# mom-ocean/MOM6

Measured on AMD Instinct MI355X. Metric: simulated-days/wall-sec, higher is better.
Workload: dtype f64

## Files before the change

### mom6_amd/abi.py

```python
import ctypes as C
import os

_HERE = os.path.dirname(os.path.abspath(__file__))
LIB_PATH = os.path.join(_HERE, "lib", "libmom6x.so")

c_double_p = C.POINTER(C.c_double)


class Dims(C.Structure):
    _fields_ = [
        ("ni", C.c_int), ("nj", C.c_int), ("nk", C.c_int), ("halo", C.c_int),
        ("ioff", C.c_int), ("joff", C.c_int), ("pitch", C.c_int), ("slab", C.c_int),
        ("i_glob0", C.c_int), ("j_glob0", C.c_int), ("ni_glob", C.c_int), ("nj_glob", C.c_int),
        ("reentrant_x", C.c_int), ("reentrant_y", C.c_int),
    ]

    @property
    def nrows(self):
        return self.nj + 2 * self.halo + 1

    def shape2(self):
        return (self.nrows, self.pitch)

    def shape3(self, nk=None):
# ... 387 lines not shown
    g_prime = np.empty(nk)
    g_prime[0] = g_Earth
    g_prime[1:] = (g_Earth / Rho0) * (Rlay[1:] - Rlay[:-1])
    return np.ascontiguousarray(Rlay), np.ascontiguousarray(g_prime)


class RK2Params(C.Structure):
    _fields_ = [("be", C.c_double), ("begw", C.c_double), ("split_bottom_stress", C.c_int),
                ("BT_use_layer_fluxes", C.c_int), ("store_CAu", C.c_int), ("visc_rem_dt_bug", C.c_int), ("remap_aux", C.c_int),
                ("no_BT_cont", C.c_int)]


def rk2_params_default():
    p = RK2Params()
    p.be, p.begw = 0.6, 0.0
    p.split_bottom_stress = 0
    p.BT_use_layer_fluxes = p.store_CAu = p.visc_rem_dt_bug = 1
    p.remap_aux = 0
    p.no_BT_cont = 0
    return p


VERTVISC_COEF_HOOK = C.CFUNCTYPE(C.c_int, C.c_void_p, C.c_int, C.c_void_p, C.c_void_p, C.c_void_p, C.c_double)
HOR_VISC_HOOK = C.CFUNCTYPE(C.c_int, C.c_void_p, C.c_void_p, C.c_void_p, C.c_void_p, C.c_void_p, C.c_void_p,
                            C.c_void_p, C.c_void_p)


class RK2Hooks(C.Structure):
    _fields_ = [("user", C.c_void_p), ("vertvisc_coef", VERTVISC_COEF_HOOK), ("horizontal_viscosity", HOR_VISC_HOOK)]


RK2_FIELDS = ["CAu", "CAv", "CAu_pred", "CAv_pred", "PFu", "PFv", "diffu", "diffv", "visc_rem_u", "visc_rem_v",
              "u_accel_bt", "v_accel_bt", "u_av", "v_av", "h_av", "pbce", "eta", "eta_PF", "uhbt", "vhbt",
              "taux_bot", "tauy_bot", "BT_h_u", "BT_h_v"]
RK2_HAVE_ETA, RK2_HAVE_DIFFU, RK2_HAVE_U2, RK2_HAVE_CAU, RK2_HAVE_UH, RK2_HAVE_H2 = 1, 2, 4, 8, 16, 32
RK2_FIELDS_2D = {"eta", "eta_PF", "uhbt", "vhbt", "taux_bot", "tauy_bot"}


METRICS = [
    "mask2dT", "mask2dCu", "mask2dCv", "mask2dBu",
    "dxT", "dyT", "IdxT", "IdyT",
    "dxCu", "dyCu", "IdxCu", "IdyCu",
    "dxCv", "dyCv", "IdxCv", "IdyCv",
    "dxBu", "dyBu", "IdxBu", "IdyBu",
    "areaT", "IareaT", "areaBu", "IareaBu",
    "areaCu", "areaCv", "IareaCu", "IareaCv",
    "dy_Cu", "dx_Cv", "bathyT", "CoriolisBu", "Coriolis2Bu",
]
G = {n: i for i, n in enumerate(METRICS)}
G_COUNT = len(METRICS)

MOM6X_OK = 0

_lib = None


ABI_VERSION = 6


def load_library(path=None):
    global _lib
    if _lib is not None and path is None:
        return _lib
    p = path or LIB_PATH
    if not os.path.exists(p):
        raise RuntimeError(
            f"mom6_amd: HIP extension {p} is missing; run `python -c 'import __graft_entry__ as g; g.build()'`. "
            "There is no CPU fallback for the product path.")
    lib = C.CDLL(p, mode=C.RTLD_GLOBAL)
# ... 24 lines not shown
```

### mom6_amd/csrc/continuity.hip

```cpp
#include "continuity_dev.h"
#include "continuity_lds.h"
#include <cstdlib>

namespace {

bool use_lds_path(int nk) {
  const char *e = getenv("MOM6X_MASSFLUX");
  if (e && !strcmp(e, "legacy")) return false;
  return mass_flux_lds_usable(nk);
}


template <int DIR>
__global__ void __launch_bounds__(256)
k_edge(Dm d, const double *__restrict__ G, const double *__restrict__ h_in, double *__restrict__ h_L,
       double *__restrict__ h_R, double h_min, int scheme , int monotonic,
       int i0, int i1, int j0, int j1) {
  const int i = i0 + blockIdx.x * blockDim.x + threadIdx.x;
  const int j = j0 + blockIdx.y * blockDim.y + threadIdx.y;
  const int k = blockIdx.z;
  if (i > i1 || j > j1) return;
  const int st = DIR ? d.pitch : 1;
  const double *m = gm(G, d, MOM6X_G_mask2dT);
  const size_t c2 = ix2(d, i, j);
// ... 244 lines not shown
  const int j = b0 + blockIdx.y * blockDim.y + threadIdx.y;
  const int k = blockIdx.z;
  if (i > a1 || j > b1) return;
  const int st = DIR ? d.pitch : 1;
  const double *IdT = gm(G, d, DIR ? MOM6X_G_IdyT : MOM6X_G_IdxT);
  const double *Lface = gm(G, d, DIR ? MOM6X_G_dx_Cv : MOM6X_G_dy_Cu), *IareaT = gm(G, d, MOM6X_G_IareaT);
  const size_t f2 = ix2(d, i, j), f = f2 + (size_t)k * d.slab, p = f + st;
  const double uf = u[f];
  double h_avg, h_marg;
  if (uf > 0.0) {
    const double CFL = vol_CFL ? (uf * dt) * (Lface[f2] * IareaT[f2]) : uf * dt * IdT[f2];
    const double curv_3 = (hL[f] + hR[f]) - 2.0 * h[f];
    h_avg = hR[f] + CFL * (0.5 * (hL[f] - hR[f]) + curv_3 * (CFL - 1.5));
    h_marg = hR[f] + CFL * ((hL[f] - hR[f]) + 3.0 * curv_3 * (CFL - 1.0));
  } else if (uf < 0.0) {
    const double CFL = vol_CFL ? (-uf * dt) * (Lface[f2] * IareaT[f2 + st]) : -uf * dt * IdT[f2 + st];
    const double curv_3 = (hL[p] + hR[p]) - 2.0 * h[p];
    h_avg = hL[p] + CFL * (0.5 * (hR[p] - hL[p]) + curv_3 * (CFL - 1.5));
    h_marg = hL[p] + CFL * ((hR[p] - hL[p]) + 3.0 * curv_3 * (CFL - 1.0));
  } else {
    h_avg = 0.5 * (hL[p] + hR[f]);
    h_marg = 0.5 * (hL[p] + hR[f]);
  }
  double hu = marginal ? h_marg : h_avg;
  if (visc_rem) hu = hu * (visc_rem[f] * 1.0);
  else hu = hu * 1.0;
  h_u[f] = hu;
}

template <int DIR>
__global__ void __launch_bounds__(256)
k_convergence(Dm d, const double *__restrict__ G, double *h, const double *__restrict__ uh, double dt,
              const double *hin, double h_min, int i0, int i1, int j0, int j1, int *flag, double *h_av, const double *av_src,
              int av_mode) {
  const int i = I_BASE(i0) + blockIdx.x * blockDim.x + threadIdx.x;
  const int j = j0 + blockIdx.y * blockDim.y + threadIdx.y;
  if (i < i0 || i > i1 || j > j1) return;
  const int st = DIR ? d.pitch : 1;
  const size_t c2 = ix2(d, i, j), slab = (size_t)d.slab;
  const double IareaT = gm(G, d, MOM6X_G_IareaT)[c2];
  const int k0 = blockIdx.z * KCHUNK, k1 = min(k0 + KCHUNK, d.nk);
  const bool own = (i >= 0 && i <= d.ni - 1 && j >= 0 && j <= d.nj - 1);
  bool bad = false;
  for (int k = k0; k < k1; k++) {
    const size_t c = c2 + (size_t)k * slab;
    const double h_old = hin[c];
    const double hn = h_old - dt * IareaT * (uh[c] - uh[c - st]);
    const double hnew = dmax(hn, h_min);
    h[c] = hnew;
    if (av_mode && own) {
      if (av_mode == 1) h_av[c] = 0.5 * (av_src[c] + hnew);
      else if (av_mode == 2) h_av[c] = h_old;
      else h_av[c] = 0.5 * (h_av[c] + hnew);
    }
    bad = bad || (hn != hn);
  }
  if (bad) atomicOr(flag, 1);
}

template <int DIR>
int run_direction(mom6x_ctx *c, const double *u, const double *h_src, double *h, double *uh, double dt,
                  int ish, int ieh, int jsh, int jeh, const double *uhbt, const double *visc_rem,
                  double *u_cor, const mom6x_BT_cont *BT, double *du_cor, const double *hin_conv,
                  double h_min_conv, bool first_pass) {
  const Dm d = c->d;
  const mom6x_continuity_params &P = c->cont;
  const dim3 blk(64, 4, 1);
  int ei0 = ish, ei1 = ieh, ej0 = jsh, ej1 = jeh;
  if (DIR == 0) { ei0 = ish - 1; ei1 = ieh + 1; } else { ej0 = jsh - 1; ej1 = jeh + 1; }
  const int scheme = P.upwind_1st ? 2 : (P.simple_2nd ? 1 : 0);
  const bool special = P.aggress_adjust || P.vol_CFL;
  const bool wave = !special && (P.sum_order == MOM6X_SUM_TREE16 || P.sum_order == MOM6X_SUM_TREE16_FMA);
  const bool lds = !special && (wave || use_lds_path(d.nk));
  if (!lds)
    KLAUNCH(c, "k_edge<DIR>", k_edge<DIR>, grid3(ei1 - ei0 + 1, ej1 - ej0 + 1, d.nk, blk), blk, d, c->G, h_src,
                       c->hL, c->hR, 2.0 * c->GV.Angstrom_H, scheme, P.monotonic, ei0, ei1, ej0, ej1);
  FluxArgs A;
  memset(&A, 0, sizeof(A));
  A.u = u; A.h_in = h_src; A.hL = c->hL; A.hR = c->hR; A.uh = uh; A.uhbt = uhbt; A.visc_rem = visc_rem;
  A.u_cor = u_cor; A.du_cor = du_cor; A.set_BT_cont = (BT != nullptr);
  if (BT) {
    if (DIR == 0) { A.FA_m0 = BT->FA_u_W0; A.FA_mm = BT->FA_u_WW; A.uBT_mm = BT->uBT_WW;
                    A.FA_p0 = BT->FA_u_E0; A.FA_pp = BT->FA_u_EE; A.uBT_pp = BT->uBT_EE; }
    else          { A.FA_m0 = BT->FA_v_S0; A.FA_mm = BT->FA_v_SS; A.uBT_mm = BT->vBT_SS;
                    A.FA_p0 = BT->FA_v_N0; A.FA_pp = BT->FA_v_NN; A.uBT_pp = BT->vBT_NN; }
  }
  A.dt = dt; A.CFL_limit_adjust = P.CFL_limit_adjust; A.tol_eta = P.tol_eta; A.tol_vel = P.tol_vel;
  A.better_iter = P.better_iter; A.use_visc_rem_max = P.use_visc_rem_max;
  A.aggress_adjust = P.aggress_adjust; A.vol_CFL = P.vol_CFL;
// ... 18 lines not shown
      FluxArgs S1 = A, S2 = A;
      S1.a0 = a0; S1.a1 = a1; S1.b0 = b0; S1.b1 = b1;
      S2.a0 = c0; S2.a1 = c1; S2.b0 = e0; S2.b1 = e1;
      return mass_flux_wave_pair(c, DIR, S1, S2, E);
    };
    int rc;
    if (!split) {
      rc = part(A.a0, A.a1, A.b0, A.b1);
    } else if (DIR == 0) {
      const int o0 = A.b0 > 0 ? A.b0 : 0, o1 = A.b1 < d.nj - 1 ? A.b1 : d.nj - 1;
      rc = part(A.a0, A.a1, o0, o1);
      halo_complete(c);
      if (!rc) rc = pair(A.a0, A.a1, A.b0, o0 - 1, A.a0, A.a1, o1 + 1, A.b1);
    } else {
      const int o0 = A.a0 > 0 ? A.a0 : 0, o1 = A.a1 < d.ni - 1 ? A.a1 : d.ni - 1;
      rc = part(o0, o1, A.b0, A.b1);
      halo_complete(c);
      if (!rc) rc = pair(A.a0, o0 - 1, A.b0, A.b1, o1 + 1, A.a1, A.b0, A.b1);
    }
    if (rc) return rc;
  } else {
    KLAUNCH(c, "k_mass_flux<DIR>", k_mass_flux<DIR>, grid3(A.a1 - A.a0 + 1, A.b1 - A.b0 + 1, 1, blk), blk, d, c->G, A);
    if (BT_h) {
      KLAUNCH(c, "k_flux_thickness<DIR>", k_flux_thickness<DIR>, grid3(A.a1 - A.a0 + 1, A.b1 - A.b0 + 1, d.nk, blk), blk,
                         d, c->G, (u_cor ? (const double *)u_cor : u), h_src, c->hL, c->hR, BT_h, dt,
                         P.marginal_faces, visc_rem, A.a0, A.a1, A.b0, A.b1, P.vol_CFL);
    }
  }
  if (first_pass || !c->cont_h_unused)
  {
    int av_mode = 0;
    if (c->cont_av_kind == 1 && !first_pass) av_mode = 1;
    if (c->cont_av_kind == 2) av_mode = first_pass ? 2 : 3;
    KLAUNCH(c, "k_convergence<DIR>", k_convergence<DIR>, grid3(nxa(ieh - ish + 1, ish), jeh - jsh + 1, nchunks(d.nk), blk), blk, d, c->G,
                       h, uh, dt, hin_conv, h_min_conv, ish, ieh, jsh, jeh, c->flag, c->cont_av, c->cont_av_src, av_mode);
  }
  HIPCHK(hipGetLastError());
  return MOM6X_OK;
}

}

extern "C" int mom6x_continuity_init(mom6x_ctx *c, const mom6x_continuity_params *p) {
  REQUIRE(c && p, MOM6X_EINVAL, "mom6x_continuity_init: null argument");
  REQUIRE(p->sum_order == MOM6X_SUM_REFERENCE || p->sum_order == MOM6X_SUM_TREE16 || p->sum_order == MOM6X_SUM_TREE16_FMA, MOM6X_EINVAL,
          "continuity_PPM: sum_order must be MOM6X_SUM_REFERENCE (0), MOM6X_SUM_TREE16 (1) or MOM6X_SUM_TREE16_FMA (2)");
  REQUIRE(p->sum_order == MOM6X_SUM_REFERENCE || mass_flux_wave_usable(c->d.nk), MOM6X_EUNSUPPORTED,
          "continuity_PPM: sum_order = MOM6X_SUM_TREE16(_FMA) carries at most 128 layers; use MOM6X_SUM_REFERENCE");
  c->cont = *p;
  c->cont_init = true;
  return MOM6X_OK;
}

extern "C" int mom6x_continuity_stats(mom6x_ctx *c, int mode, unsigned long long *out3) {
  REQUIRE(c, MOM6X_EINVAL, "mom6x_continuity_stats: null context");
  const int reset = (mode == 1);
  if (mode == 1) c->cont_stats_on = true;
  if (mode == 0) c->cont_stats_on = false;
  HIPCHK(hipSetDevice(c->device));
  if (!c->cont_stats) {
    HIPCHK(hipMalloc(&c->cont_stats, 4 * sizeof(unsigned long long)));
    HIPCHK(hipMemsetAsync(c->cont_stats, 0, 4 * sizeof(unsigned long long), c->stream));
  }
  HIPCHK(hipStreamSynchronize(c->stream));
  if (out3) HIPCHK(hipMemcpy(out3, c->cont_stats, 3 * sizeof(unsigned long long), hipMemcpyDeviceToHost));
  if (reset) HIPCHK(hipMemsetAsync(c->cont_stats, 0, 4 * sizeof(unsigned long long), c->stream));
  return MOM6X_OK;
}
// ... 35 lines not shown
```

### mom6_amd/csrc/dyn_split_RK2.hip

```cpp
#include <algorithm>
#include <cstring>
#include "mom6x_dev.h"

void halo_wrap(mom6x_ctx *c, double *const *fields, const int *staggers, const int *nks, int n);

struct RK2State {
  mom6x_rk2_params P;
  double *CAu, *CAv, *CAu_pred, *CAv_pred, *PFu, *PFv, *diffu, *diffv, *visc_rem_u, *visc_rem_v;
  double *u_accel_bt, *v_accel_bt, *u_av, *v_av, *h_av, *pbce;
  double *eta, *eta_PF, *uhbt, *vhbt, *taux_bot, *tauy_bot;
  mom6x_BT_cont BT;
  bool CAu_pred_stored;
  bool accel_bt_deferred;
  double *up, *vp, *hp, *u_bc_accel, *v_bc_accel, *uh_in, *vh_in, *eta_pred, *eta_h;
};

namespace {

__global__ void __launch_bounds__(256)
k_bc_accel(Dm d, const double *__restrict__ G, const double *__restrict__ CAu, const double *__restrict__ CAv,
           const double *__restrict__ PFu, const double *__restrict__ PFv, const double *__restrict__ diffu,
           const double *__restrict__ diffv, double *__restrict__ u_bc, double *__restrict__ v_bc,
           const double *__restrict__ u, const double *__restrict__ v, double *__restrict__ up, double *__restrict__ vp,
           double dt) {
// ... 160 lines not shown
}

extern "C" int mom6x_initialize_dyn_split_RK2(mom6x_ctx *c, const mom6x_rk2_params *p) {
  REQUIRE(c && p, MOM6X_EINVAL, "mom6x_initialize_dyn_split_RK2: null argument");
  REQUIRE(c->cont_init && c->bt_init && c->cor_init && c->pgf_init, MOM6X_EINVAL,
          "initialize_dyn_split_RK2: continuity, barotropic, CoriolisAdv and PressureForce must be initialised first");
  REQUIRE(!p->remap_aux || p->store_CAu, MOM6X_EINVAL, "REMAP_AUXILIARY_VARS requires that STORE_CORIOLIS_ACCEL = True.");
  REQUIRE(p->BT_use_layer_fluxes && p->store_CAu, MOM6X_EUNSUPPORTED,
          "dyn_split_RK2: only BT_USE_LAYER_FLUXES=True and STORE_CORIOLIS_ACCEL=True are supported");
  HIPCHK(hipSetDevice(c->device));
  if (c->rk2) rk2_state_free(c);
  RK2State *s = new RK2State();
  memset(s, 0, sizeof(*s));
  s->P = *p;
  const size_t n2 = (size_t)c->dims.slab, n3 = n2 * c->dims.nk;
  double **p3[] = { &s->CAu, &s->CAv, &s->CAu_pred, &s->CAv_pred, &s->PFu, &s->PFv, &s->diffu, &s->diffv, &s->visc_rem_u,
                    &s->visc_rem_v, &s->u_accel_bt, &s->v_accel_bt, &s->u_av, &s->v_av, &s->h_av, &s->pbce, &s->up, &s->vp,
                    &s->hp, &s->u_bc_accel, &s->v_bc_accel, &s->uh_in, &s->vh_in, &s->BT.h_u, &s->BT.h_v };
  for (double **q : p3) { HIPCHK(hipMalloc(q, n3 * sizeof(double))); HIPCHK(hipMemsetAsync(*q, 0, n3 * sizeof(double), c->stream)); }
  double **p2[] = { &s->eta, &s->eta_PF, &s->uhbt, &s->vhbt, &s->taux_bot, &s->tauy_bot, &s->eta_pred, &s->eta_h, &s->BT.FA_u_EE,
                    &s->BT.FA_u_E0, &s->BT.FA_u_W0, &s->BT.FA_u_WW, &s->BT.uBT_WW, &s->BT.uBT_EE, &s->BT.FA_v_NN, &s->BT.FA_v_N0,
                    &s->BT.FA_v_S0, &s->BT.FA_v_SS, &s->BT.vBT_SS, &s->BT.vBT_NN };
  for (double **q : p2) { HIPCHK(hipMalloc(q, n2 * sizeof(double))); HIPCHK(hipMemsetAsync(*q, 0, n2 * sizeof(double), c->stream)); }
  s->CAu_pred_stored = false;
  c->rk2 = s;
  return MOM6X_OK;
}

extern "C" double *mom6x_rk2_field(mom6x_ctx *c, int which) {
  if (!c || !c->rk2) return nullptr;
  RK2State *s = c->rk2;
  double *t[] = { s->CAu, s->CAv, s->CAu_pred, s->CAv_pred, s->PFu, s->PFv, s->diffu, s->diffv, s->visc_rem_u, s->visc_rem_v,
                  s->u_accel_bt, s->v_accel_bt, s->u_av, s->v_av, s->h_av, s->pbce, s->eta, s->eta_PF, s->uhbt, s->vhbt,
                  s->taux_bot, s->tauy_bot, s->BT.h_u, s->BT.h_v };
  if (which < 0 || which >= (int)(sizeof(t) / sizeof(t[0]))) return nullptr;
  if ((which == 10 || which == 11) && s->accel_bt_deferred) {
    if (hipSetDevice(c->device) != hipSuccess) return nullptr;
    if (bt_layer_accel_materialize(c, s->u_accel_bt, s->v_accel_bt) != MOM6X_OK) return nullptr;
    if (hipStreamSynchronize(c->stream) != hipSuccess) return nullptr;
    s->accel_bt_deferred = false;
  }
  return t[which];
}

extern "C" int mom6x_rk2_set_CAu_pred_stored(mom6x_ctx *c, int stored) {
  REQUIRE(c && c->rk2, MOM6X_EINVAL, "mom6x_rk2_set_CAu_pred_stored: dyn_split_RK2 not initialised");
  c->rk2->CAu_pred_stored = (stored != 0);
  return MOM6X_OK;
}

#define CHK(call) do { int rc_ = (call); if (rc_) return rc_; } while (0)

extern "C" int mom6x_remap_dyn_split_RK2_aux_vars(mom6x_ctx *c, const mom6x_remapping_params *p, const double *h_old_u,
                                                  const double *h_old_v, const double *h_new_u, const double *h_new_v) {
  REQUIRE(c && c->rk2, MOM6X_EINVAL, "remap_dyn_split_RK2_aux_vars: dyn_split_RK2 not initialised");
  RK2State *s = c->rk2;
  if (!s->P.remap_aux) return MOM6X_OK;
  if (s->P.store_CAu) {
    CHK(mom6x_ALE_remap_velocities(c, p, h_old_u, h_old_v, h_new_u, h_new_v, s->u_av, s->v_av));
    CHK(pass3(c, {s->u_av, s->v_av}, {1, 2}, c->d.nk));
    CHK(mom6x_ALE_remap_velocities(c, p, h_old_u, h_old_v, h_new_u, h_new_v, s->CAu_pred, s->CAv_pred));
    CHK(pass3(c, {s->CAu_pred, s->CAv_pred}, {1, 2}, c->d.nk));
  }
  CHK(mom6x_ALE_remap_velocities(c, p, h_old_u, h_old_v, h_new_u, h_new_v, s->diffu, s->diffv));
  REQUIRE(!c->halo_error, MOM6X_EHIP, mom6x_last_error());
  return MOM6X_OK;
}
// ... 119 lines not shown
  if (calc_dtbt) CHK(set_dtbt_eta(c, s->pbce, BTp ? nullptr : eta));
  const bool defer_la = dev_coef && !host_coef;
  bt_defer_layer_accel(c, defer_la);
  s->accel_bt_deferred = defer_la;
  LayerAccelSrc LAu, LAv;
  CHK(mom6x_btstep(c, u_inst, v_inst, eta, dt, u_bc, v_bc, taux, tauy, s->pbce, s->eta_PF, u_av, v_av, s->u_accel_bt,
                   s->v_accel_bt, s->eta_pred, s->uhbt, s->vhbt, s->visc_rem_u, s->visc_rem_v, BTp, taux_bot, tauy_bot,
                   s->uh_in, s->vh_in, u_inst, v_inst, nullptr));

  const double dt_pred = dt * R.be;
  if (!host_coef) {
    const bool same_dt = (R.visc_rem_dt_bug != 0);
    if (defer_la) REQUIRE(bt_layer_accel_src(c, &LAu, &LAv), MOM6X_EINVAL, "step_MOM_dyn_split_RK2: no barotropic result to take the layer accelerations from");
    CHK(vertvisc_stage_solve(c, u_inst, v_inst, u_bc, v_bc, s->u_accel_bt, s->v_accel_bt, defer_la ? &LAu : nullptr, defer_la ? &LAv : nullptr,
                             dt_pred, h, up, vp, taux, tauy, s->taux_bot, s->tauy_bot,
                             same_dt ? s->visc_rem_u : nullptr, same_dt ? s->visc_rem_v : nullptr,
                             !same_dt ));
    if (!same_dt) CHK(mom6x_vertvisc_remnant(c, s->visc_rem_u, s->visc_rem_v, dt));
  } else {
    KLAUNCH(c, "k_vel_update", k_vel_update, gridk(nxa(d.ni + 1, -1), d.nj + 1, nk, b), b, d, c->G, (const double *)u_inst,
            (const double *)v_inst, u_bc, v_bc, s->u_accel_bt, s->v_accel_bt, up, vp, dt_pred);
    CHK(coef_hook(1, up, vp, dt_pred));
    if (R.visc_rem_dt_bug) {
      CHK(vertvisc_fused(c, nullptr, nullptr, nullptr, nullptr, nullptr, nullptr, 0.0, up, vp, taux, tauy, dt_pred, s->taux_bot,
                         s->tauy_bot, s->visc_rem_u, s->visc_rem_v));
    } else {
      CHK(mom6x_vertvisc(c, up, vp, taux, tauy, dt_pred, s->taux_bot, s->tauy_bot));
      CHK(mom6x_vertvisc_remnant(c, s->visc_rem_u, s->visc_rem_v, dt));
    }
  }
  start3(c, { s->visc_rem_u, s->visc_rem_v, up, vp }, { 1, 2, 1, 2 }, nk, { PW.cont, PW.cont, PW.cont, PW.cont });

  c->cont_av_kind = 1; c->cont_av = h_av; c->cont_av_src = h;
  {
    const int rc_c = mom6x_continuity_PPM(c, up, vp, h, hp, uh, vh, dt, s->uhbt, s->vhbt, s->visc_rem_u, s->visc_rem_v, u_av, v_av, BTp,
                                          nullptr, nullptr);
    c->cont_av_kind = 0;
    if (rc_c) return rc_c;
  }
  halo_complete(c);
  start3(c, { hp, u_av, v_av, uh, vh }, { 0, 1, 2, 1, 2 }, nk, { PW.vel ? 2 : 0, PW.vel, PW.vel, PW.vel, PW.vel });

  CHK(mom6x_bt_mass_source(c, hp, s->eta_pred, 0));
  halo_complete(c);
  KLAUNCH(c, "k_h_av", k_h_av, gridk(nxa(d.ni + 4, -2), d.nj + 4, nk, b), b, d, h_av, (const double *)h, (const double *)hp, 0, 0.0, 2, 2);
  if (R.begw != 0.0) {
    KLAUNCH(c, "k_h_av", k_h_av, gridk(nxa(d.ni + 2, -1), d.nj + 2, nk, b), b, d, hp, (const double *)h, (const double *)nullptr, 3, R.begw, 1, 0);
    CHK(mom6x_PressureForce(c, hp, s->PFu, s->PFv, s->pbce, s->eta_PF));
  }
  if (BTp) {
    bt_defer_btcalc(c, true);
    CHK(mom6x_btcalc(c, h, s->BT.h_u, s->BT.h_v));
  }
  if (hooks && hooks->horizontal_viscosity) {
    HIPCHK(hipStreamSynchronize(c->stream));
    int rc = hooks->horizontal_viscosity(hooks->user, u_av, v_av, h_av, uh, vh, s->diffu, s->diffv);
    REQUIRE(rc == 0, MOM6X_EINVAL, "step_MOM_dyn_split_RK2: horizontal_viscosity callback failed");
  } else if (c->hv_init) {
    CHK(mom6x_horizontal_viscosity(c, u_av, v_av, h_av, s->diffu, s->diffv));
  }
  CHK(CorAdCalc_bc(c, u_av, v_av, h_av, uh, vh, s->CAu, s->CAv, s->PFu, s->PFv, s->diffu, s->diffv, u_bc, v_bc, nullptr, nullptr, 0.0));
  CHK(mom6x_btstep(c, u_inst, v_inst, eta, dt, u_bc, v_bc, taux, tauy, s->pbce, s->eta_PF, u_av, v_av, s->u_accel_bt,
                   s->v_accel_bt, s->eta_pred, s->uhbt, s->vhbt, s->visc_rem_u, s->visc_rem_v, BTp, taux_bot, tauy_bot, uh, vh,
                   u_av, v_av, eta_av));
  KLAUNCH(c, "k_eta", k_eta, grid3(d.ni, d.nj, 1, b), b, d, c->G, eta, (const double *)s->eta_pred, (const double *)nullptr, 0.0);
  if (!host_coef) {
    if (defer_la) REQUIRE(bt_layer_accel_src(c, &LAu, &LAv), MOM6X_EINVAL, "step_MOM_dyn_split_RK2: no barotropic result to take the layer accelerations from");
    CHK(vertvisc_stage_solve(c, u_inst, v_inst, u_bc, v_bc, s->u_accel_bt, s->v_accel_bt, defer_la ? &LAu : nullptr, defer_la ? &LAv : nullptr,
                             dt, h, u_inst, v_inst, taux, tauy, s->taux_bot, s->tauy_bot, s->visc_rem_u, s->visc_rem_v, true));
  } else {
    KLAUNCH(c, "k_vel_update", k_vel_update, gridk(nxa(d.ni + 1, -1), d.nj + 1, nk, b), b, d, c->G, (const double *)u_inst,
            (const double *)v_inst, u_bc, v_bc, s->u_accel_bt, s->v_accel_bt, u_inst, v_inst, dt);
    CHK(coef_hook(2, u_inst, v_inst, dt));
    CHK(vertvisc_fused(c, nullptr, nullptr, nullptr, nullptr, nullptr, nullptr, 0.0, u_inst, v_inst, taux, tauy, dt, s->taux_bot,
                       s->tauy_bot, s->visc_rem_u, s->visc_rem_v));
  }
// ... 22 lines not shown
```

### mom6_amd/csrc/mom6x_dev.h

```cpp
#pragma once
#include <hip/hip_runtime.h>
#include <cstdio>
#include <cstring>
#include <string>
#include "../../include/mom6x.h"

struct Dm {
  int ni, nj, nk, halo, ioff, joff, pitch, slab;
};

__host__ __device__ inline Dm make_dm(const mom6x_dims &d) {
  Dm m; m.ni = d.ni; m.nj = d.nj; m.nk = d.nk; m.halo = d.halo; m.ioff = d.ioff; m.joff = d.joff;
  m.pitch = d.pitch; m.slab = d.slab; return m;
}

__device__ __forceinline__ size_t ix2(const Dm &d, int i, int j) {
  return (size_t)(i + d.ioff) + (size_t)(j + d.joff) * (size_t)d.pitch;
}
__device__ __forceinline__ size_t ix3(const Dm &d, int i, int j, int k) {
  return ix2(d, i, j) + (size_t)k * (size_t)d.slab;
}
__device__ __forceinline__ const double *gm(const double *G, const Dm &d, int m) {
  return G + (size_t)m * (size_t)d.slab;
}
// ... 33 lines not shown
  int first_direction;
  mom6x_continuity_params cont; bool cont_init;
  mom6x_barotropic_params bt; bool bt_init;
  double *hL, *hR;
  int *retry; size_t retry_cap;
  BTState *bts;
  RK2State *rk2;
  int *flag;
  mom6x_coriolis_params cor; bool cor_init;
  mom6x_pgf_params pgf; bool pgf_init;
  double *Rlay, *g_prime;
  const double *tv_T, *tv_S; mom6x_eos_params eos;
  const double *a_u, *a_v, *h_u, *h_v, *Ray_u, *Ray_v;
  mom6x_vertvisc_params vv; bool vv_init;
  const double *Kv_bbl_u, *Kv_bbl_v, *bbl_thick_u, *bbl_thick_v, *Kv_shear;
  double *vv_a_u, *vv_a_v, *vv_h_u, *vv_h_v;
  mom6x_hor_visc_params hv; bool hv_init; double *hv_planes;
  double ds_Hmix; const double *ds_h;
  double *regrid_res;
  double *remap_hvel;
  double *remap_src;
  double *regrid_vec;
  double *scr[MOM6X_NSCR]; int scr_nlev[MOM6X_NSCR];
  bool prof_on;
  struct Prof *prof;
  void *ta;
  long long *red; size_t red_cap;
  void *diag;
  void *comm;
  bool bt_overlap;
  bool halo_error;
  hipEvent_t ev_ready, ev_done; bool pass_pending;
  int cont_av_kind; double *cont_av; const double *cont_av_src;
  int pass_w = 0, dyn_pass_width = 0;
  int pass_wf[16] = {0}, pass_wf_n = 0;
  long long n_exchanges = 0, n_exchange_bytes = 0;
  BcFold pgf_fold = { nullptr, nullptr, nullptr, nullptr, nullptr, nullptr, nullptr };
  bool pgf_eta_h_written = false;
  bool cont_stats_on;
  unsigned long long *cont_stats;
  bool cont_h_unused;
  mom6x_set_visc_params sv; bool sv_init = false; bool sv_use_eos = false; mom6x_eos_params sv_eos; const double *sv_tideamp = nullptr;
  mom6x_thickness_diffuse_params td; bool td_init = false; bool td_use_eos = false; mom6x_eos_params td_eos;
  const double *td_khth2d = nullptr; double *td_work = nullptr;
  void *thd = nullptr;
  void *vm = nullptr;
};
void thickness_diffuse_free(mom6x_ctx *c);
void tracer_hor_diff_free(mom6x_ctx *c);
void varmix_free(mom6x_ctx *c);
void comm_free(mom6x_ctx *c);
void halo_start(mom6x_ctx *c, double *const *fields, const int *staggers, const int *nks, int n);
void halo_complete(mom6x_ctx *c);
bool halo_start_packed(mom6x_ctx *c, double *const *fields, const int *staggers, const int *nks, int n);
bool halo_can_overlap(const mom6x_ctx *c);
int comm_allreduce_scalar(mom6x_ctx *c, double *value, int op);

void prof_begin(mom6x_ctx *c, const char *name);
void prof_end(mom6x_ctx *c);
#define KLAUNCH(c, name, kern, grid, blk, ...)                              \
  do {                                                                      \
    if ((c)->prof_on) prof_begin((c), name);                                \
    hipLaunchKernelGGL(kern, grid, blk, 0, (c)->stream, __VA_ARGS__);       \
    if ((c)->prof_on) prof_end((c));                                        \
  } while (0)

// ... 58 lines not shown
```

### mom6_amd/csrc/pressure_force.hip

```cpp
#include "mom6x_dev.h"
#include "eos_dev.h"

namespace {

__global__ void __launch_bounds__(256)
k_pgf_e(Dm d, const double *__restrict__ G, const double *__restrict__ h, double *__restrict__ e, double H_to_Z) {
  const int i = I_BASE(-1) + blockIdx.x * blockDim.x + threadIdx.x;
  const int j = -1 + blockIdx.y * blockDim.y + threadIdx.y;
  if (i > d.ni || j > d.nj) return;
  if (i < (-1)) return;
  const size_t x = ix2(d, i, j), slab = (size_t)d.slab;
  double ek = -gm(G, d, MOM6X_G_bathyT)[x];
  e[x + (size_t)d.nk * slab] = ek;
  for (int k = d.nk - 1; k >= 0; k--) {
    ek = ek + h[x + (size_t)k * slab] * H_to_Z;
    e[x + (size_t)k * slab] = ek;
  }
}

__global__ void __launch_bounds__(256)
k_pgf_main(Dm d, const double *__restrict__ G, const double *__restrict__ h, const double *__restrict__ e,
           const double *__restrict__ Rlay, const double *__restrict__ g_prime, double *__restrict__ PFu,
           double *__restrict__ PFv, double *__restrict__ pbce, double *__restrict__ eta, double g_Earth,
           double H_to_Z, double Z_to_H, double rho_ref, double GxRho_ref, double Z_ref, double I_Rho0,
           double h_neglect, double dz_neglect, BcFold B) {
  const int i = I_BASE(-1) + blockIdx.x * blockDim.x + threadIdx.x;
  const int j = -1 + blockIdx.y * blockDim.y + threadIdx.y;
  if (i > d.ni || j > d.nj) return;
  if (i < (-1)) return;
  const int st = d.pitch, nz = d.nk;
  const size_t x = ix2(d, i, j), slab = (size_t)d.slab;
  const bool do_u = (i <= d.ni - 1) && (j >= 0) && (j <= d.nj - 1);
// ... 18 lines not shown
    const double eb0 = e[cb];
    if (do_u) {
      const double h1 = h[c + 1];
      const double dz1 = g_Earth * H_to_Z * h1;
      const double iz1 = 0.5 * R * dz1 * h1;
      const double intx_dpa = 0.5 * R * (dz0 + dz1);
      const double pf = (((pa0 * h0 + iz0) - (pa1 * h1 + iz1)) + ((h1 - h0) * intx_pa - (e[cb + 1] - eb0) * intx_dpa * Z_to_H)) *
                        (cu / ((h0 + h1) + h_neglect));
      PFu[c] = pf;
      if (B.u_bc) B.u_bc[c] = (B.CAu[c] + pf) + B.diffu[c];
      pa1 = pa1 + R * dz1;
      intx_pa = intx_pa + intx_dpa;
    }
    if (do_v) {
      const double h2 = h[c + st];
      const double dz2 = g_Earth * H_to_Z * h2;
      const double iz2 = 0.5 * R * dz2 * h2;
      const double inty_dpa = 0.5 * R * (dz0 + dz2);
      const double pf = (((pa0 * h0 + iz0) - (pa2 * h2 + iz2)) + ((h2 - h0) * inty_pa - (e[cb + st] - eb0) * inty_dpa * Z_to_H)) *
                        (cv / ((h0 + h2) + h_neglect));
      PFv[c] = pf;
      if (B.v_bc) B.v_bc[c] = (B.CAv[c] + pf) + B.diffv[c];
      pa2 = pa2 + R * dz2;
      inty_pa = inty_pa + inty_dpa;
    }
    pa0 = pa0 + dpa0;
    if (pbce) {
      if (k == 0) pb = g_prime[0] * H_to_Z;
      else pb = pb + (g_prime[k] * H_to_Z) * ((e[c] - e_bot) * Ihtot);
      pbce[c] = pb;
    }
  }
  if (do_eh) B.eta_h[x] = eta_h;
}

}

struct EosDev { int form; double Rho_T0_S0, dRho_dT, dRho_dS, dRho_dp; int do_mw, top_mw, ssh_z0; int van_only; double dz_nv; };

namespace {

template <int FORM>
__device__ __forceinline__ void cell_int(const EosDev &E, double rho_ref, double G_e, double GxRho, double I_Rho, double T,
                                         double S, double zt, double zb, double z0, double &dpa, double &intz) {
  const double dz = zt - zb;
  const double p_ave = -GxRho * (0.5 * (zt + zb) - z0);
  if (FORM == MOM6X_EOS_LINEAR) {
    const double C1_6 = 1.0 / 6.0;
    const double rho_anom = (E.Rho_T0_S0 - rho_ref) + E.dRho_dT * T + E.dRho_dS * S + E.dRho_dp * p_ave;
    dpa = G_e * rho_anom * dz;
    intz = 0.5 * G_e * (rho_anom - C1_6 * E.dRho_dp * (GxRho * dz)) * (dz * dz);
  } else {
    const double C1_3 = 1.0 / 3.0, C1_7 = 1.0 / 7.0, C1_9 = 1.0 / 9.0;
    double al0, p0, lambda;
    wright_coefs<FORM>(T, S, al0, p0, lambda);
    const double I_al0 = 1.0 / al0;
    if (FORM == MOM6X_EOS_WRIGHT) {
      const double I_Lzz = 1.0 / (p0 + (lambda * I_al0) + p_ave);
      const double eps = 0.5 * GxRho * dz * I_Lzz, eps2 = eps * eps;
      const double rho_anom = (p0 + p_ave) * (I_Lzz * I_al0) - rho_ref;
      const double rem = I_Rho * (lambda * (I_al0 * I_al0)) * eps2 * (C1_3 + eps2 * (0.2 + eps2 * (C1_7 + C1_9 * eps2)));
      dpa = 1.0 * (G_e * rho_anom * dz - 2.0 * eps * rem);
      intz = 1.0 * (0.5 * G_e * rho_anom * (dz * dz) - dz * (1.0 + eps) * rem);
    } else {
      const double I_Lzz = 1.0 / ((p0 + p_ave) + lambda * I_al0);
      const double eps = 0.5 * (GxRho * dz) * I_Lzz, eps2 = eps * eps;
// ... 388 lines not shown
  REQUIRE(c, MOM6X_EINVAL, "mom6x_PressureForce_set_tv: null ctx");
  if (!T) { c->tv_T = nullptr; c->tv_S = nullptr; return MOM6X_OK; }
  REQUIRE(S && eos, MOM6X_EINVAL, "mom6x_PressureForce_set_tv: tv%T without tv%S or tv%eqn_of_state");
  REQUIRE(eos->form >= MOM6X_EOS_LINEAR && eos->form <= MOM6X_EOS_ROQUET_SPV, MOM6X_EUNSUPPORTED,
          "PressureForce: EQN_OF_STATE must be LINEAR, WRIGHT, WRIGHT_FULL, WRIGHT_REDUCED, UNESCO, ROQUET_RHO (NEMO), JACKETT_06 or ROQUET_SPV");
  REQUIRE(eos->form < MOM6X_EOS_UNESCO || eos->EOS_quadrature || eos->Recon_Scheme, MOM6X_EUNSUPPORTED,
          "No analytic integration option is available with this EOS!");
  REQUIRE(eos->Recon_Scheme >= 0 && eos->Recon_Scheme <= 2, MOM6X_EINVAL,
          "PressureForce_FV_init: PRESSURE_RECONSTRUCTION_SCHEME must be 1 (PLM) or 2 (PPM), or 0 without RECONSTRUCT_FOR_PRESSURE");
  REQUIRE(eos->Recon_Scheme != 2 || c->dims.nk >= 4, MOM6X_EUNSUPPORTED,
          "PressureForce_FV: PRESSURE_RECONSTRUCTION_SCHEME = 2 (edge_values_implicit_h4) needs NK >= 4");
  c->tv_T = T; c->tv_S = S; c->eos = *eos;
  return MOM6X_OK;
}

extern "C" int mom6x_PressureForce_init(mom6x_ctx *c, const mom6x_pgf_params *p, const double *Rlay, const double *g_prime) {
  REQUIRE(c && p && Rlay && g_prime, MOM6X_EINVAL, "mom6x_PressureForce_init: null argument");
  HIPCHK(hipSetDevice(c->device));
  c->pgf = *p;
  const size_t n = (size_t)c->dims.nk * sizeof(double);
  if (!c->Rlay) { HIPCHK(hipMalloc(&c->Rlay, n)); HIPCHK(hipMalloc(&c->g_prime, n)); }
  HIPCHK(hipMemcpy(c->Rlay, Rlay, n, hipMemcpyHostToDevice));
  HIPCHK(hipMemcpy(c->g_prime, g_prime, n, hipMemcpyHostToDevice));
  c->pgf_init = true;
  return MOM6X_OK;
}

extern "C" int mom6x_PressureForce(mom6x_ctx *c, const double *h, double *PFu, double *PFv, double *pbce, double *eta) {
  REQUIRE(c && c->pgf_init, MOM6X_EINVAL, "MOM_PressureForce_FV_Bouss: Module must be initialized before it is used.");
  REQUIRE(h && PFu && PFv, MOM6X_EINVAL, "PressureForce: null array");
  HIPCHK(hipSetDevice(c->device));
  c->pgf_eta_h_written = false;
  const Dm d = c->d;
  double *e;
  int rc;
  if ((rc = ctx_scratch(c, SCR_e, d.nk + 1, &e))) return rc;
  const dim3 b = blk2();
  const mom6x_vgrid &GV = c->GV;
  const double GxRho0 = GV.g_Earth * GV.Rho0;
  const double GxRho_ref = c->pgf.rho_ref_bug ? GxRho0 : GV.g_Earth * c->pgf.rho_ref;
  KLAUNCH(c, "k_pgf_e", k_pgf_e, grid3(nxa(d.ni + 2, -1), d.nj + 2, 1, b), b, d, c->G, h, e, GV.H_to_Z);
  if (c->tv_T) {
    EosDev E;
    E.form = c->eos.form; E.Rho_T0_S0 = c->eos.Rho_T0_S0; E.dRho_dT = c->eos.dRho_dT; E.dRho_dS = c->eos.dRho_dS;
    E.dRho_dp = c->eos.dRho_dp; E.do_mw = c->eos.MassWghtInterp & 1; E.top_mw = (c->eos.MassWghtInterp >> 1) & 1;
    E.ssh_z0 = c->eos.use_SSH_in_Z0p;
    E.van_only = c->eos.MassWghtInterpVanOnly; E.dz_nv = GV.H_to_Z * c->eos.h_nonvanished;
    const double rho0_alt = c->pgf.rho_ref_bug ? c->pgf.rho_ref : GV.Rho0;
    const dim3 g = grid3(nxa(d.ni + 2, -1), d.nj + 2, 1, b);
    const int mode = c->eos.Recon_Scheme ? c->eos.Recon_Scheme : (c->eos.EOS_quadrature ? 3 : 0);
    double *Tt = nullptr, *Tb = nullptr, *St = nullptr, *Sb = nullptr;
    if (mode == 1 || mode == 2) {
      if ((rc = ctx_scratch(c, SCR_t0, d.nk, &Tt)) || (rc = ctx_scratch(c, SCR_t1, d.nk, &Tb)) ||
          (rc = ctx_scratch(c, SCR_t2, d.nk, &St)) || (rc = ctx_scratch(c, SCR_t3, d.nk, &Sb))) return rc;
      if (mode == 1) {
        if ((rc = mom6x_ALE_PLM_edge_values(c, h, c->tv_S, c->eos.boundary_extrap, St, Sb))) return rc;
        if ((rc = mom6x_ALE_PLM_edge_values(c, h, c->tv_T, c->eos.boundary_extrap, Tt, Tb))) return rc;
      } else {
        if ((rc = mom6x_ALE_PPM_edge_values(c, h, c->tv_S, c->eos.boundary_extrap, St, Sb))) return rc;
        if ((rc = mom6x_ALE_PPM_edge_values(c, h, c->tv_T, c->eos.boundary_extrap, Tt, Tb))) return rc;
      }
    }
#define PGF_EOS(F, P, NAME) KLAUNCH(c, NAME, (k_pgf_main_eos<F, P>), g, b, d, c->G, h, e, c->tv_T, c->tv_S, Tt, Tb, St, Sb, E, PFu, PFv,   \
                                    pbce, eta, GV.g_Earth, GV.H_to_Z, GV.Z_to_H, c->pgf.rho_ref, GxRho_ref, c->pgf.Z_ref, GV.Rho0, \
                                    rho0_alt, GV.H_subroundoff, GV.dZ_subroundoff, c->pgf_fold)
#define PGF_FORM(F, N) do { if (mode == 1) PGF_EOS(F, 1, "k_pgf_main_plm<" N ">"); else if (mode == 2) PGF_EOS(F, 2, "k_pgf_main_ppm<" N ">"); \
                            else if (mode == 3) PGF_EOS(F, 3, "k_pgf_main_pcm<" N ">"); else PGF_EOS(F, 0, "k_pgf_main_eos<" N ">"); } while (0)
    if (E.form == MOM6X_EOS_UNESCO) {
      if (mode == 1) PGF_EOS(MOM6X_EOS_UNESCO, 1, "k_pgf_main_plm<unesco>");
      else if (mode == 2) PGF_EOS(MOM6X_EOS_UNESCO, 2, "k_pgf_main_ppm<unesco>");
      else PGF_EOS(MOM6X_EOS_UNESCO, 3, "k_pgf_main_pcm<unesco>");
    } else if (E.form == MOM6X_EOS_ROQUET_RHO) {
      if (mode == 1) PGF_EOS(MOM6X_EOS_ROQUET_RHO, 1, "k_pgf_main_plm<roquet_rho>");
// ... 27 lines not shown
```

Baseline: 0.1928.

## Fuse interface-height build into column PGF kernel and eta_h into continuity convergence

For the no-temperature (layered) pressure-force case, a new column-per-thread kernel builds interface heights in registers and computes PFu/PFv/pbce/eta (and optionally the folded bc accelerations and eta_h) in one pass. Within each wavefront, east-neighbour data comes from lane shuffles, and a readlane seam handles the lane that has no east neighbour in the same wavefront. This replaces the separate k_pgf_e pass and its scratch array. The predictor continuity convergence also accumulates the column sum eta_h, so the barotropic mass source can be built from it instead of rereading hp. The costs are heavy register use for per-column arrays, a single k-chunk in convergence (less parallelism), and inline-asm fragility.

```diff
diff --git a/mom6_amd/abi.py b/mom6_amd/abi.py
--- a/mom6_amd/abi.py
+++ b/mom6_amd/abi.py
@@ -443,9 +443,9 @@
 
 RK2_FIELDS = ["CAu", "CAv", "CAu_pred", "CAv_pred", "PFu", "PFv", "diffu", "diffv", "visc_rem_u", "visc_rem_v",
               "u_accel_bt", "v_accel_bt", "u_av", "v_av", "h_av", "pbce", "eta", "eta_PF", "uhbt", "vhbt",
-              "taux_bot", "tauy_bot", "BT_h_u", "BT_h_v"]
+              "taux_bot", "tauy_bot", "BT_h_u", "BT_h_v", "u_bc_accel", "v_bc_accel", "eta_pred", "eta_h"]
 RK2_HAVE_ETA, RK2_HAVE_DIFFU, RK2_HAVE_U2, RK2_HAVE_CAU, RK2_HAVE_UH, RK2_HAVE_H2 = 1, 2, 4, 8, 16, 32
-RK2_FIELDS_2D = {"eta", "eta_PF", "uhbt", "vhbt", "taux_bot", "tauy_bot"}
+RK2_FIELDS_2D = {"eta", "eta_PF", "uhbt", "vhbt", "taux_bot", "tauy_bot", "eta_pred", "eta_h"}
 
 
 METRICS = [
diff --git a/mom6_amd/csrc/continuity.hip b/mom6_amd/csrc/continuity.hip
--- a/mom6_amd/csrc/continuity.hip
+++ b/mom6_amd/csrc/continuity.hip
@@ -300,15 +300,17 @@
 __global__ void __launch_bounds__(256)
 k_convergence(Dm d, const double *__restrict__ G, double *h, const double *__restrict__ uh, double dt,
               const double *hin, double h_min, int i0, int i1, int j0, int j1, int *flag, double *h_av, const double *av_src,
-              int av_mode) {
+              int av_mode, int kchunk, double *__restrict__ eta_h, double Z_to_H) {
   const int i = I_BASE(i0) + blockIdx.x * blockDim.x + threadIdx.x;
   const int j = j0 + blockIdx.y * blockDim.y + threadIdx.y;
   if (i < i0 || i > i1 || j > j1) return;
   const int st = DIR ? d.pitch : 1;
   const size_t c2 = ix2(d, i, j), slab = (size_t)d.slab;
   const double IareaT = gm(G, d, MOM6X_G_IareaT)[c2];
-  const int k0 = blockIdx.z * KCHUNK, k1 = min(k0 + KCHUNK, d.nk);
+  const int k0 = blockIdx.z * kchunk, k1 = min(k0 + kchunk, d.nk);
   const bool own = (i >= 0 && i <= d.ni - 1 && j >= 0 && j <= d.nj - 1);
+  const bool do_eh = (eta_h != nullptr) && own;
+  double eh = 0.0;
   bool bad = false;
   for (int k = k0; k < k1; k++) {
     const size_t c = c2 + (size_t)k * slab;
@@ -316,6 +318,7 @@
     const double hn = h_old - dt * IareaT * (uh[c] - uh[c - st]);
     const double hnew = dmax(hn, h_min);
     h[c] = hnew;
+    if (do_eh) eh = (k == 0) ? (hnew - gm(G, d, MOM6X_G_bathyT)[c2] * Z_to_H) : (eh + hnew);
     if (av_mode && own) {
       if (av_mode == 1) h_av[c] = 0.5 * (av_src[c] + hnew);
       else if (av_mode == 2) h_av[c] = h_old;
@@ -323,6 +326,7 @@
     }
     bad = bad || (hn != hn);
   }
+  if (do_eh) eta_h[c2] = eh;
   if (bad) atomicOr(flag, 1);
 }
 
@@ -407,8 +411,12 @@
     int av_mode = 0;
     if (c->cont_av_kind == 1 && !first_pass) av_mode = 1;
     if (c->cont_av_kind == 2) av_mode = first_pass ? 2 : 3;
-    KLAUNCH(c, "k_convergence<DIR>", k_convergence<DIR>, grid3(nxa(ieh - ish + 1, ish), jeh - jsh + 1, nchunks(d.nk), blk), blk, d, c->G,
-                       h, uh, dt, hin_conv, h_min_conv, ish, ieh, jsh, jeh, c->flag, c->cont_av, c->cont_av_src, av_mode);
+    double *eta_h = (av_mode == 1) ? c->cont_eta_h : nullptr;
+    const int kchunk = eta_h ? d.nk : KCHUNK;
+    KLAUNCH(c, "k_convergence<DIR>", k_convergence<DIR>, grid3(nxa(ieh - ish + 1, ish), jeh - jsh + 1, eta_h ? 1 : nchunks(d.nk), blk), blk, d, c->G,
+                       h, uh, dt, hin_conv, h_min_conv, ish, ieh, jsh, jeh, c->flag, c->cont_av, c->cont_av_src, av_mode, kchunk, eta_h,
+                       c->GV.Z_to_H);
+    if (eta_h) c->cont_eta_h_written = true;
   }
   HIPCHK(hipGetLastError());
   return MOM6X_OK;
diff --git a/mom6_amd/csrc/dyn_split_RK2.hip b/mom6_amd/csrc/dyn_split_RK2.hip
--- a/mom6_amd/csrc/dyn_split_RK2.hip
+++ b/mom6_amd/csrc/dyn_split_RK2.hip
@@ -216,7 +216,7 @@
   RK2State *s = c->rk2;
   double *t[] = { s->CAu, s->CAv, s->CAu_pred, s->CAv_pred, s->PFu, s->PFv, s->diffu, s->diffv, s->visc_rem_u, s->visc_rem_v,
                   s->u_accel_bt, s->v_accel_bt, s->u_av, s->v_av, s->h_av, s->pbce, s->eta, s->eta_PF, s->uhbt, s->vhbt,
-                  s->taux_bot, s->tauy_bot, s->BT.h_u, s->BT.h_v };
+                  s->taux_bot, s->tauy_bot, s->BT.h_u, s->BT.h_v, s->u_bc_accel, s->v_bc_accel, s->eta_pred, s->eta_h };
   if (which < 0 || which >= (int)(sizeof(t) / sizeof(t[0]))) return nullptr;
   if ((which == 10 || which == 11) && s->accel_bt_deferred) {
     if (hipSetDevice(c->device) != hipSuccess) return nullptr;
@@ -402,16 +402,21 @@
   start3(c, { s->visc_rem_u, s->visc_rem_v, up, vp }, { 1, 2, 1, 2 }, nk, { PW.cont, PW.cont, PW.cont, PW.cont });
 
   c->cont_av_kind = 1; c->cont_av = h_av; c->cont_av_src = h;
+  c->cont_eta_h = ms_own ? nullptr : s->eta_h; c->cont_eta_h_written = false;
+  bool have_eta_hp = false;
   {
     const int rc_c = mom6x_continuity_PPM(c, up, vp, h, hp, uh, vh, dt, s->uhbt, s->vhbt, s->visc_rem_u, s->visc_rem_v, u_av, v_av, BTp,
                                           nullptr, nullptr);
     c->cont_av_kind = 0;
+    have_eta_hp = c->cont_eta_h_written;
+    c->cont_eta_h = nullptr; c->cont_eta_h_written = false;
     if (rc_c) return rc_c;
   }
   halo_complete(c);
   start3(c, { hp, u_av, v_av, uh, vh }, { 0, 1, 2, 1, 2 }, nk, { PW.vel ? 2 : 0, PW.vel, PW.vel, PW.vel, PW.vel });
 
-  CHK(mom6x_bt_mass_source(c, hp, s->eta_pred, 0));
+  if (have_eta_hp) CHK(bt_mass_source_from(c, s->eta_h, s->eta_pred, 0));
+  else CHK(mom6x_bt_mass_source(c, hp, s->eta_pred, 0));
   halo_complete(c);
   KLAUNCH(c, "k_h_av", k_h_av, gridk(nxa(d.ni + 4, -2), d.nj + 4, nk, b), b, d, h_av, (const double *)h, (const double *)hp, 0, 0.0, 2, 2);
   if (R.begw != 0.0) {
diff --git a/mom6_amd/csrc/mom6x_dev.h b/mom6_amd/csrc/mom6x_dev.h
--- a/mom6_amd/csrc/mom6x_dev.h
+++ b/mom6_amd/csrc/mom6x_dev.h
@@ -89,6 +89,7 @@
   bool halo_error;
   hipEvent_t ev_ready, ev_done; bool pass_pending;
   int cont_av_kind; double *cont_av; const double *cont_av_src;
+  double *cont_eta_h = nullptr; bool cont_eta_h_written = false;
   int pass_w = 0, dyn_pass_width = 0;
   int pass_wf[16] = {0}, pass_wf_n = 0;
   long long n_exchanges = 0, n_exchange_bytes = 0;
diff --git a/mom6_amd/csrc/pressure_force.hip b/mom6_amd/csrc/pressure_force.hip
--- a/mom6_amd/csrc/pressure_force.hip
+++ b/mom6_amd/csrc/pressure_force.hip
@@ -1,3 +1,4 @@
+#include <utility>
 #include "mom6x_dev.h"
 #include "eos_dev.h"
 
@@ -82,6 +83,175 @@
     }
   }
   if (do_eh) B.eta_h[x] = eta_h;
+}
+
+template <int... Is, class F>
+__device__ __forceinline__ void static_for_seq(std::integer_sequence<int, Is...>, F &&f) { (f(std::integral_constant<int, Is>{}), ...); }
+template <int N, class F>
+__device__ __forceinline__ void static_for(F &&f) { static_for_seq(std::make_integer_sequence<int, N>{}, f); }
+
+template <int NKT, bool FOLD>
+__global__ void __launch_bounds__(64)
+k_pgf_main_cols(Dm d, const double *__restrict__ G, const double *__restrict__ h, const double *__restrict__ Rlay,
+                const double *__restrict__ g_prime, double *__restrict__ PFu, double *__restrict__ PFv, double *__restrict__ pbce,
+                double *__restrict__ eta, double g_Earth, double H_to_Z, double Z_to_H, double rho_ref, double GxRho_ref, double Z_ref,
+                double I_Rho0, double h_neglect, double dz_neglect, BcFold B) {
+  constexpr int NK = NK_OF(NKT);
+  const int nk = NK_EXACT(NKT) ? NK : d.nk;
+  const int lane = threadIdx.x;
+  const int ib = I_BASE(-1) + blockIdx.x * 64;
+  const int i = ib + lane, j = -1 + blockIdx.y;
+  const bool live = (i >= -1) && (i <= d.ni);
+  const int ic = min(max(i, -1), d.ni);
+  const size_t slab = (size_t)d.slab;
+  const unsigned x = (unsigned)ix2(d, ic, j) * 8u;
+  const unsigned xn = (unsigned)ix2(d, ic, min(j + 1, d.nj)) * 8u;
+  const unsigned xe = (unsigned)ix2(d, min(ic + 1, d.ni), j) * 8u;
+  unsigned xs = (unsigned)ix2(d, min(ib + 64, d.ni), j) * 8u;
+  asm volatile("v_mov_b32 %0, %1" : "=v"(xs) : "s"(xs));
+  auto at = [](const double *base, unsigned off) -> const double & { return *(const double *)((const char *)base + off); };
+  auto to = [](double *base, unsigned off) -> double & { return *(double *)((char *)base + off); };
+  const bool do_u = live && (i <= d.ni - 1) && (j >= 0) && (j <= d.nj - 1);
+  const bool do_v = (j <= d.nj - 1) && (i >= 0) && (i <= d.ni - 1);
+  const double *bathyT = gm(G, d, MOM6X_G_bathyT);
+
+  double eA[NK + 1], eN[NK + 1];
+  int seam_lo0 = 0, seam_hi0 = 0, seam_lo1 = 0, seam_hi1 = 0;
+  auto seam_put = [&](auto kc, double v) {
+    constexpr int k = decltype(kc)::value;
+    int lo = (k < 64) ? seam_lo0 : seam_lo1, hi = (k < 64) ? seam_hi0 : seam_hi1;
+    asm("v_writelane_b32 %0, %1, %2" : "+v"(lo) : "s"(__builtin_amdgcn_readfirstlane(__double2loint(v))), "n"(k & 63));
+    asm("v_writelane_b32 %0, %1, %2" : "+v"(hi) : "s"(__builtin_amdgcn_readfirstlane(__double2hiint(v))), "n"(k & 63));
+    if (k < 64) { seam_lo0 = lo; seam_hi0 = hi; } else { seam_lo1 = lo; seam_hi1 = hi; }
+  };
+  auto seam_get = [&](int k) {
+    return __hiloint2double(__builtin_amdgcn_readlane((k < 64) ? seam_hi0 : seam_hi1, k & 63),
+                            __builtin_amdgcn_readlane((k < 64) ? seam_lo0 : seam_lo1, k & 63));
+  };
+  const double depth = at(bathyT, x), e_bot = -depth;
+  double ea = e_bot, en = -at(bathyT, xn), es = -at(bathyT, xs);
+  eA[NK] = ea; eN[NK] = en; seam_put(std::integral_constant<int, NK>{}, es);
+  {
+    constexpr int PG = NK_EXACT(NKT) ? 4 : 3, NG = (NK + PG - 1) / PG;
+    double q_a[2][PG], q_n[2][PG], q_s[2][PG];
+    const double *hk = h + (size_t)(nk - 1) * slab;
+    auto fetch = [&](int g, int b) {
+#pragma unroll
+      for (int m = 0; m < PG; m++) {
+        const int k = NK - 1 - (g * PG + m);
+        if (k >= 0) {
+          q_a[b][m] = at(hk, x); q_n[b][m] = at(hk, xn); q_s[b][m] = at(hk, xs);
+          if (k > 0) hk -= (NK_EXACT(NKT) || k <= nk - 1) ? slab : (size_t)0;
+        }
+      }
+    };
+    fetch(0, 0);
+    static_for<NG>([&](auto gc) {
+      constexpr int g = decltype(gc)::value;
+      if (g + 1 < NG) fetch(g + 1, (g + 1) & 1);
+      __builtin_amdgcn_sched_barrier(0);
+      static_for<PG>([&](auto mc) {
+        constexpr int k = NK - 1 - (g * PG + decltype(mc)::value);
+        if constexpr (k >= 0) {
+          if (NK_EXACT(NKT) || k < nk) {
+            ea = ea + q_a[g & 1][decltype(mc)::value] * H_to_Z;
+            en = en + q_n[g & 1][decltype(mc)::value] * H_to_Z;
+            es = es + q_s[g & 1][decltype(mc)::value] * H_to_Z;
+          }
+          eA[k] = ea; eN[k] = en; seam_put(std::integral_constant<int, k>{}, es);
+        }
+      });
+      __builtin_amdgcn_sched_barrier(0);
+    });
+  }
+  auto east = [&](int k) { const double v = __shfl_down(eA[k], 1, 64); return (lane == 63) ? seam_get(k) : v; };
+
+  const double e_top = eA[0];
+  if (eta && live) to(eta, x) = e_top * Z_to_H;
+  const double Ihtot = 1.0 / ((e_top - e_bot) + dz_neglect);
+  double pa0 = GxRho_ref * (e_top - Z_ref), pa1 = 0.0, pa2 = 0.0, intx_pa = 0.0, inty_pa = 0.0;
+  double cu = 0.0, cv = 0.0;
+  const double e_top_e = east(0);
+  if (do_u) { pa1 = GxRho_ref * (e_top_e - Z_ref); intx_pa = 0.5 * (pa0 + pa1); cu = (2.0 * I_Rho0 * at(gm(G, d, MOM6X_G_IdxCu), x)); }
+  if (do_v) { pa2 = GxRho_ref * (eN[0] - Z_ref); inty_pa = 0.5 * (pa0 + pa2); cv = (2.0 * I_Rho0 * at(gm(G, d, MOM6X_G_IdyCv), x)); }
+  double pb = 0.0;
+  const bool do_eh = (B.eta_h != nullptr) && i >= 0 && i <= d.ni - 1 && j >= 0 && j <= d.nj - 1;
+  double eta_h = 0.0;
+  constexpr int TG = NK_EXACT(NKT) ? (FOLD ? 3 : 4) : ((FOLD && NK % 3 == 0) ? 4 : 3), NT = (NK + TG - 1) / TG;
+  double q_0[2][TG], q_1[2][TG], q_2[2][TG], q_cu[2][TG], q_du[2][TG], q_cv[2][TG], q_dv[2][TG];
+  double q_R[2][TG], q_g[2][TG];
+  size_t kin = 0, kout = 0;
+  int nk2 = nk;
+  if (!NK_EXACT(NKT)) asm volatile("" : "+s"(nk2));
+  auto fetch = [&](int g, int b) {
+#pragma unroll
+    for (int m = 0; m < TG; m++) {
+      const int k = g * TG + m;
+      if (k < NK) {
+        q_R[b][m] = Rlay[NK_EXACT(NKT) ? k : min(k, nk2 - 1)]; q_g[b][m] = g_prime[NK_EXACT(NKT) ? k : min(k, nk2 - 1)];
+        q_0[b][m] = at(h + kin, x); q_1[b][m] = at(h + kin, xe); q_2[b][m] = at(h + kin, xn);
+        if (FOLD) { q_cu[b][m] = at(B.CAu + kin, x); q_du[b][m] = at(B.diffu + kin, x); q_cv[b][m] = at(B.CAv + kin, x); q_dv[b][m] = at(B.diffv + kin, x); }
+        kin += (NK_EXACT(NKT) || k < nk2 - 1) ? slab : (size_t)0;
+      }
+    }
+  };
+  fetch(0, 0);
+#pragma unroll
+  for (int g = 0; g < NT; g++) {
+    if (g + 1 < NT) fetch(g + 1, (g + 1) & 1);
+    __builtin_amdgcn_sched_barrier(0);
+#pragma unroll
+    for (int m = 0; m < TG; m++) {
+      const int k = g * TG + m;
+      if (k < NK && (NK_EXACT(NKT) || k < nk2)) {
+        const double R = q_R[g & 1][m] - rho_ref;
+        const double h0 = q_0[g & 1][m];
+        if (do_eh) eta_h = (k == 0) ? (h0 - depth * Z_to_H) : (eta_h + h0);
+        const double dz0 = g_Earth * H_to_Z * h0;
+        const double dpa0 = R * dz0, iz0 = 0.5 * R * dz0 * h0;
+        const double eb0 = eA[k + 1];
+        const double eb1 = east(k + 1);
+        if (do_u) {
+          const double h1 = q_1[g & 1][m];
+          const double dz1 = g_Earth * H_to_Z * h1;
+          const double iz1 = 0.5 * R * dz1 * h1;
+          const double intx_dpa = 0.5 * R * (dz0 + dz1);
+          const double pf = (((pa0 * h0 + iz0) - (pa1 * h1 + iz1)) + ((h1 - h0) * intx_pa - (eb1 - eb0) * intx_dpa * Z_to_H)) *
+                            (cu / ((h0 + h1) + h_neglect));
+          to(PFu + kout, x) = pf;
+          if (FOLD) to(B.u_bc + kout, x) = (q_cu[g & 1][m] + pf) + q_du[g & 1][m];
+          pa1 = pa1 + R * dz1;
+          intx_pa = intx_pa + intx_dpa;
+        }
+        if (do_v) {
+          const double h2 = q_2[g & 1][m];
+          const double dz2 = g_Earth * H_to_Z * h2;
+          const double iz2 = 0.5 * R * dz2 * h2;
+          const double inty_dpa = 0.5 * R * (dz0 + dz2);
+          const double pf = (((pa0 * h0 + iz0) - (pa2 * h2 + iz2)) + ((h2 - h0) * inty_pa - (eN[k + 1] - eb0) * inty_dpa * Z_to_H)) *
+                            (cv / ((h0 + h2) + h_neglect));
+          to(PFv + kout, x) = pf;
+          if (FOLD) to(B.v_bc + kout, x) = (q_cv[g & 1][m] + pf) + q_dv[g & 1][m];
+          pa2 = pa2 + R * dz2;
+          inty_pa = inty_pa + inty_dpa;
+        }
+        pa0 = pa0 + dpa0;
+        if (pbce) {
+          if (k == 0) pb = q_g[g & 1][m] * H_to_Z;
+          else pb = pb + (q_g[g & 1][m] * H_to_Z) * ((eA[k] - e_bot) * Ihtot);
+          if (live) to(pbce + kout, x) = pb;
+        }
+        kout += slab;
+      }
+    }
+    __builtin_amdgcn_sched_barrier(0);
+  }
+  if (do_eh) to(B.eta_h, x) = eta_h;
+}
+
+bool pgf_pair() {
+  static const bool pair = [] { const char *e = getenv("MOM6X_PGF"); return e && !strcmp(e, "pair"); }();
+  return pair;
 }
 
 }
@@ -536,13 +706,28 @@
   HIPCHK(hipSetDevice(c->device));
   c->pgf_eta_h_written = false;
   const Dm d = c->d;
+  const mom6x_vgrid &GV = c->GV;
+  const double GxRho0 = GV.g_Earth * GV.Rho0;
+  const double GxRho_ref = c->pgf.rho_ref_bug ? GxRho0 : GV.g_Earth * c->pgf.rho_ref;
+  if (!c->tv_T && d.nk <= COLS_NK_BOUND && (size_t)d.slab * sizeof(double) < ((size_t)1 << 32) && !pgf_pair()) {
+    const dim3 bc(64, 1, 1), gc((unsigned)((nxa(d.ni + 2, -1) + 63) / 64), (unsigned)(d.nj + 2), 1);
+    const bool fold = (c->pgf_fold.u_bc != nullptr);
+#define PGC(NKT) do { if (fold) KLAUNCH(c, "k_pgf_main_cols", (k_pgf_main_cols<NKT, true>), gc, bc, d, c->G, h, c->Rlay, c->g_prime, PFu, PFv,   \
+                                        pbce, eta, GV.g_Earth, GV.H_to_Z, GV.Z_to_H, c->pgf.rho_ref, GxRho_ref, c->pgf.Z_ref, 1.0 / GV.Rho0,       \
+                                        GV.H_subroundoff, GV.dZ_subroundoff, c->pgf_fold);                                                        \
+                      else KLAUNCH(c, "k_pgf_main_cols", (k_pgf_main_cols<NKT, false>), gc, bc, d, c->G, h, c->Rlay, c->g_prime, PFu, PFv,        \
+                                   pbce, eta, GV.g_Earth, GV.H_to_Z, GV.Z_to_H, c->pgf.rho_ref, GxRho_ref, c->pgf.Z_ref, 1.0 / GV.Rho0,            \
+                                   GV.H_subroundoff, GV.dZ_subroundoff, c->pgf_fold); } while (0)
+    COLS_NK_DISPATCH(d.nk, PGC);
+#undef PGC
+    c->pgf_eta_h_written = (c->pgf_fold.eta_h != nullptr);
+    HIPCHK(hipGetLastError());
+    return MOM6X_OK;
+  }
   double *e;
   int rc;
   if ((rc = ctx_scratch(c, SCR_e, d.nk + 1, &e))) return rc;
   const dim3 b = blk2();
-  const mom6x_vgrid &GV = c->GV;
-  const double GxRho0 = GV.g_Earth * GV.Rho0;
-  const double GxRho_ref = c->pgf.rho_ref_bug ? GxRho0 : GV.g_Earth * c->pgf.rho_ref;
   KLAUNCH(c, "k_pgf_e", k_pgf_e, grid3(nxa(d.ni + 2, -1), d.nj + 2, 1, b), b, d, c->G, h, e, GV.H_to_Z);
   if (c->tv_T) {
     EosDev E;
```

Result: faster. 0.1954 (median of 6 runs) (+1.3%).
